# venomouscyanide/S3GRL

Hardware: AMD Instinct MI355X
Metric: link-pair precomputes/sec (higher is better)
Workload: dtype f32; 1 GPU; pubmed_pos_k3; mode=pos, sign_k=3, num_hops=3, num_nodes=19717, features=500, graph=real topology, synthetic features (BASELINE.md §3)

## Files before the change

### s3grl_amd/csrc/s3grl_packed.hip

```cpp
#include <algorithm>
#include <cstdlib>
#include <type_traits>

#include "s3grl_internal.hpp"
#include "s3grl_gather_common.hpp"

namespace s3grl {
namespace {


constexpr int kTile = 512;
constexpr int kWavesPerBlock = 1;

__device__ __forceinline__ int below(uint64_t m) {
  return __builtin_amdgcn_mbcnt_hi((uint32_t)(m >> 32), __builtin_amdgcn_mbcnt_lo((uint32_t)m, 0u));
}

__device__ __forceinline__ float4_t dense_chunk(const float* __restrict__ X, int64_t ld, int F, int64_t row,
                                                int tile, int j) {
  const int col = tile * kTile + j * 4;
  if (col >= F) return (float4_t)(0.f);
  float4_t v = *reinterpret_cast<const float4_t*>(X + row * ld + col);
  if (col + 1 >= F) v.y = 0.f;
  if (col + 2 >= F) v.z = 0.f;
  if (col + 3 >= F) v.w = 0.f;
  return v;
}

__device__ __forceinline__ bool nonzero(float4_t v) {
  return v.x != 0.f || v.y != 0.f || v.z != 0.f || v.w != 0.f;
}

__global__ __launch_bounds__(256) void pk_count_kernel(const float* __restrict__ X, int64_t ld, int F,
                                                       int64_t N, int tiles, int32_t* __restrict__ cnt) {
  const int lane = threadIdx.x & 63;
  const int64_t item = (int64_t)blockIdx.x * 4 + (threadIdx.x >> 6);
  if (item >= N * tiles) return;
  const int tile = (int)(item / N);
  const int64_t row = item - (int64_t)tile * N;
  const uint64_t m0 = __ballot(nonzero(dense_chunk(X, ld, F, row, tile, lane)));
  const uint64_t m1 = __ballot(nonzero(dense_chunk(X, ld, F, row, tile, 64 + lane)));
  if (lane == 0) cnt[item] = __popcll(m0) + __popcll(m1);
}

__global__ __launch_bounds__(256) void pk_fill_kernel(const float* __restrict__ X, int64_t ld, int F,
                                                      int64_t N, int tiles, const int64_t* __restrict__ ptr,
                                                      PackedHdr* __restrict__ hdr,
                                                      float4_t* __restrict__ data) {
  const int lane = threadIdx.x & 63;
  const int64_t item = (int64_t)blockIdx.x * 4 + (threadIdx.x >> 6);
  if (item >= N * tiles) return;
  const int tile = (int)(item / N);
  const int64_t row = item - (int64_t)tile * N;
  const float4_t v0 = dense_chunk(X, ld, F, row, tile, lane);
  const float4_t v1 = dense_chunk(X, ld, F, row, tile, 64 + lane);
  const uint64_t m0 = __ballot(nonzero(v0));
  const uint64_t m1 = __ballot(nonzero(v1));
  const int64_t off = ptr[item] + 1;
  if (item == 0 && lane == 0) data[0] = (float4_t)(0.f);
  if ((m0 >> lane) & 1) data[off + below(m0)] = v0;
  if ((m1 >> lane) & 1) data[off + __popcll(m0) + below(m1)] = v1;
  if (lane == 0) {
    PackedHdr h;
    h.m0 = m0;
    h.m1 = m1;
    h.off = (uint64_t)off;
    h.el = 0;
    hdr[item] = h;
  }
}

typedef unsigned int uint4_t __attribute__((ext_vector_type(4)));
constexpr uint32_t kOobOffset = 0x80000000u;

__device__ __forceinline__ uint32_t select_or_oob(uint64_t mask, uint32_t if_set, uint32_t oob) {
  uint32_t r;
  asm("v_cndmask_b32_e64 %0, %3, %1, %2" : "=v"(r) : "v"(if_set), "s"(mask), "v"(oob));
  return r;
}

template <int K>
__device__ __forceinline__ int el_phase_b_start(const int (&lim)[K], int cnt) {
  constexpr int U = 4;
  int nb = 1;
#pragma unroll
  for (int i = K - 2; i >= 0; --i)
    if (lim[i] == lim[K - 1] && nb == K - 1 - i) nb = K - i;
  if (nb != 1) return cnt;
  const int ngf = cnt / U;
  const int limA = K >= 2 ? lim[K >= 2 ? K - 2 : 0] : 0;
  const int gA = min(ngf, (limA + U - 1) / U);
  return gA < ngf ? gA * U : cnt;
}

typedef unsigned int uint2_t __attribute__((ext_vector_type(2)));

template <int K>
__device__ __forceinline__ void el_phase_b(const Job* __restrict__ jobs, int njobs, const int32_t* __restrict__ c_ids,
                                           const float* __restrict__ c_coef, const float* __restrict__ job_z,
                                           const int32_t* __restrict__ job_lim, const int32_t* __restrict__ job_order,
                                           const PackedHdr* __restrict__ hdr, const ElemEntry* __restrict__ el,
                                           uint32_t el_bytes, int64_t N, const float* __restrict__ X, int64_t ldx,
                                           int F, float* __restrict__ rows_out, float* __restrict__ prows) {
  constexpr int CH = 2;
  constexpr int U = 4;
  constexpr int W = 64;
  const int lane = threadIdx.x & 63;
  const int wid = __builtin_amdgcn_readfirstlane(blockIdx.x * kWavesPerBlock + (threadIdx.x >> 6));
  if (wid >= njobs) return;
  const int jid = __builtin_amdgcn_readfirstlane(job_order[wid]);
  const Job job = jobs[jid];
  if (job.split == 1) return;
  const int cnt = __builtin_amdgcn_readfirstlane(job.support);
  int lim[K];
#pragma unroll
  for (int i = 0; i < K; ++i) lim[i] = __builtin_amdgcn_readfirstlane(job_lim[(int64_t)jid * K + i]);
  const int j0 = el_phase_b_start<K>(lim, cnt);
  if (j0 >= cnt) return;
  float* __restrict__ rows = job.split == 2 ? prows : rows_out;
  const int col0 = blockIdx.y * kTile;
  const int Fp = F + 1;
  const int64_t rstride = (int64_t)(K + 1) * Fp;
  const int nrow = job.node_b >= 0 ? 2 : 1;
  int coff[CH];
  bool cok[CH];
#pragma unroll
  for (int c = 0; c < CH; ++c) {
    coff[c] = col0 + (lane + 64 * c) * 4;
    cok[c] = coff[c] < F;
  }
  float4_t acc[K][2][CH];
#pragma unroll
  for (int i = 0; i < K; ++i)
#pragma unroll
    for (int r = 0; r < 2; ++r)
#pragma unroll
      for (int c = 0; c < CH; ++c) acc[i][r][c] = (float4_t)(0.f);
#pragma unroll
  for (int r = 0; r < 2; ++r) {
    if (r >= nrow) break;
    const float* __restrict__ src = rows + (job.out_row + r) * rstride + (int64_t)K * Fp + 1;
#pragma unroll
    for (int c = 0; c < CH; ++c) {
      if (cok[c]) {
        const int nv = min(4, F - coff[c]);
        if (nv == 4) {
          acc[K - 1][r][c] = *reinterpret_cast<const float4_u*>(src + coff[c]);
        } else {
#pragma unroll
          for (int e = 0; e < 4; ++e)
            if (e < nv) acc[K - 1][r][c][e] = src[coff[c] + e];
        }
      }
    }
  }
  __shared__ __attribute__((aligned(16))) float2 el_lds[2 + kTile];
  float2* const eacc = el_lds + 1;
#pragma unroll
  for (int c = 0; c < CH; ++c)
#pragma unroll
    for (int e = 0; e < 4; ++e) eacc[1 + (lane + 64 * c) * 4 + e] = make_float2(acc[K - 1][0][c][e], acc[K - 1][1][c][e]);
  __syncthreads();

  const uint32_t* __restrict__ uid = reinterpret_cast<const uint32_t*>(c_ids + job.ids_off);
  const float2* __restrict__ cq = reinterpret_cast<const float2*>(c_coef) + job.coef_off + (int64_t)(K - 1) * cnt;
  const PackedHdr* __restrict__ th = hdr + (int64_t)blockIdx.y * N;
  const __amdgpu_buffer_rsrc_t ersrc =
      __builtin_amdgcn_make_buffer_rsrc(const_cast<ElemEntry*>(el), 0, (int)el_bytes, 0x00020000);
  const uint32_t oobv = kOobOffset;
  auto load_e = [&](uint32_t s, uint32_t k, uint32_t n) __attribute__((always_inline)) {
    const uint32_t a = (s + k + (uint32_t)lane) << 3;
    return __builtin_bit_cast(uint2_t, __builtin_amdgcn_raw_buffer_load_b64(
                                           ersrc, (int)(k + (uint32_t)lane < n ? a : oobv), 0, 0));
  };
  auto rmw = [&](uint2_t e, float qx, float qy) __attribute__((always_inline)) {
    float2 a = eacc[e.y];
    const float v = __builtin_bit_cast(float, e.x);
    a.x += qx * v;
    a.y += qy * v;
    eacc[e.y] = a;
  };
  struct EBuf {
    uint2_t e[U];
    uint32_t s[U];
    uint32_t n[U];
  };
  uint32_t idn = j0 + lane < cnt ? uid[j0 + lane] : 0u;
  for (int w0 = j0; w0 < cnt; w0 += W) {
    const int nw = min(W, cnt - w0);
    const bool mine = lane < nw;
    const uint64_t rg = mine ? th[idn].el : 0ull;
    const float2 q = mine ? cq[w0 + lane] : make_float2(0.f, 0.f);
    if (w0 + W + lane < cnt) idn = uid[w0 + W + lane];
    const uint32_t es = (uint32_t)rg, en = (uint32_t)(rg >> 32);
    const int ng = (nw + U - 1) / U;
    auto issue = [&](int g, EBuf& b) __attribute__((always_inline)) {
#pragma unroll
      for (int u = 0; u < U; ++u) {
        const int j = g * U + u;
        const int l = min(j, W - 1);
        b.s[u] = (uint32_t)__builtin_amdgcn_readlane((int)es, l);
        b.n[u] = j < W ? (uint32_t)__builtin_amdgcn_readlane((int)en, l) : 0u;
        b.e[u] = load_e(b.s[u], 0u, b.n[u]);
      }
      __builtin_amdgcn_sched_barrier(0);
    };
    auto rmw_grp = [&](int g, const EBuf& b) __attribute__((always_inline)) {
#pragma unroll
      for (int u = 0; u < U; ++u) {
        const int l = min(g * U + u, W - 1);
        const float qx = __builtin_bit_cast(float, __builtin_amdgcn_readlane(__builtin_bit_cast(int, q.x), l));
        const float qy = __builtin_bit_cast(float, __builtin_amdgcn_readlane(__builtin_bit_cast(int, q.y), l));
        rmw(b.e[u], qx, qy);
        if (__builtin_expect(b.n[u] > 64, 0)) {
#pragma nounroll
          for (uint32_t k = 64; k < b.n[u]; k += 64)
            rmw(load_e(b.s[u], k, b.n[u]), qx, qy);
        }
      }
      __builtin_amdgcn_sched_barrier(0);
    };
    EBuf bA, bB;
    issue(0, bA);
    for (int g = 0; g < ng; g += 2) {
      issue(g + 1, bB);
      rmw_grp(g, bA);
      if (g + 1 < ng) {
        issue(g + 2, bA);
        rmw_grp(g + 1, bB);
      }
    }
  }
  __syncthreads();
#pragma unroll
  for (int c = 0; c < CH; ++c)
#pragma unroll
    for (int e = 0; e < 4; ++e) {
      const float2 a = eacc[1 + (lane + 64 * c) * 4 + e];
      acc[K - 1][0][c][e] = a.x;
      acc[K - 1][1][c][e] = a.y;
    }
  write_pair_rows_part<K, CH, K - 1, K, false, true>(job, jid, acc, coff, cok, job_z, X, ldx, F, rows,
                                                     blockIdx.y == 0);
}

template <int K, int MINNB, int EL>
__global__ __launch_bounds__(kWavesPerBlock * 64) void gather_packed_kernel(
    const Job* __restrict__ jobs, int njobs, const int32_t* __restrict__ c_ids,
    const float* __restrict__ c_coef, const float* __restrict__ job_z,
    const int32_t* __restrict__ job_lim, const int32_t* __restrict__ job_order,
    const PackedHdr* __restrict__ hdr,
    const float4_t* __restrict__ data, uint32_t data_bytes, const ElemEntry* __restrict__ el, uint32_t el_bytes,
    int64_t N, const float* __restrict__ X, int64_t ldx, int F, float* __restrict__ rows_out,
    float* __restrict__ prows) {
  if constexpr (EL == 3) {
    el_phase_b<K>(jobs, njobs, c_ids, c_coef, job_z, job_lim, job_order, hdr, el, el_bytes, N, X, ldx, F, rows_out,
                  prows);
    return;
  }
  constexpr int CH = 2;
  constexpr int U = 4;
  const int lane = threadIdx.x & 63;
  const int wid = __builtin_amdgcn_readfirstlane(blockIdx.x * kWavesPerBlock + (threadIdx.x >> 6));
  if (wid >= njobs) return;
  const int jid = __builtin_amdgcn_readfirstlane(job_order[wid]);
  const int col0 = blockIdx.y * kTile;
  const Job job = jobs[jid];
  if (job.split == 1) return;
  float* __restrict__ rows = job.split == 2 ? prows : rows_out;
  const int cnt = __builtin_amdgcn_readfirstlane(job.support);
  const uint32_t* __restrict__ uid = reinterpret_cast<const uint32_t*>(c_ids + job.ids_off);
  const float2* __restrict__ cf = reinterpret_cast<const float2*>(c_coef) + job.coef_off;
  const PackedHdr* __restrict__ th = hdr + (int64_t)blockIdx.y * N;
  const __amdgpu_buffer_rsrc_t rsrc =
      __builtin_amdgcn_make_buffer_rsrc(const_cast<float4_t*>(data), 0, (int)data_bytes, 0x00020000);
  const uint32_t oobv = kOobOffset;
  int lim[K];
#pragma unroll
  for (int i = 0; i < K; ++i) lim[i] = __builtin_amdgcn_readfirstlane(job_lim[(int64_t)jid * K + i]);

  int coff[CH];
  bool cok[CH];
#pragma unroll
  for (int c = 0; c < CH; ++c) {
    coff[c] = col0 + (lane + 64 * c) * 4;
    cok[c] = coff[c] < F;
  }
  float4_t acc[K][2][CH];
#pragma unroll
  for (int i = 0; i < K; ++i)
#pragma unroll
    for (int r = 0; r < 2; ++r)
#pragma unroll
      for (int c = 0; c < CH; ++c) acc[i][r][c] = (float4_t)(0.f);

  auto hdr_of = [&](uint32_t id) __attribute__((always_inline)) -> PackedHdr {
    static_assert(sizeof(PackedHdr) == 32, "the shift below");
    return *reinterpret_cast<const PackedHdr*>(reinterpret_cast<const char*>(th) + (id << 5));
  };
  auto load_hdrs = [&](int g, PackedHdr(&h)[U]) __attribute__((always_inline)) {
    uint32_t id[U];
#pragma unroll
    for (int u = 0; u < U; ++u) id[u] = uid[g * U + u];
    __builtin_amdgcn_sched_barrier(0);
#pragma unroll
    for (int u = 0; u < U; ++u) h[u] = hdr_of(id[u]);
    __builtin_amdgcn_sched_barrier(0);
  };
  auto load_ids = [&](int g, uint32_t(&id)[U]) __attribute__((always_inline)) {
#pragma unroll
    for (int u = 0; u < U; ++u) id[u] = uid[g * U + u];
    __builtin_amdgcn_sched_barrier(0);
  };
  auto hdrs_from = [&](const uint32_t(&id)[U], PackedHdr(&h)[U]) __attribute__((always_inline)) {
#pragma unroll
    for (int u = 0; u < U; ++u) h[u] = hdr_of(id[u]);
    __builtin_amdgcn_sched_barrier(0);
  };
  auto hdrs_from_late = [&](const uint32_t(&id)[U], PackedHdr(&h)[U]) __attribute__((always_inline)) {
    uint32_t idv[U];
#pragma unroll
    for (int u = 0; u < U; ++u) idv[u] = id[u];
    asm volatile("" : "+s"(idv[0]), "+s"(idv[1]), "+s"(idv[2]), "+s"(idv[3]));
    static_assert(U == 4, "the opaque statement above lists four ids");
#pragma unroll
    for (int u = 0; u < U; ++u) h[u] = hdr_of(idv[u]);
    __builtin_amdgcn_sched_barrier(0);
  };
  auto issue = [&](const PackedHdr(&h)[U], float4_t(&v)[U][CH], bool valid = true) __attribute__((always_inline)) {
#pragma unroll
    for (int u = 0; u < U; ++u) {
      const uint32_t base = valid ? (uint32_t)h[u].off : (kOobOffset >> 4);
      const uint32_t a0 = (base + (uint32_t)below(h[u].m0)) << 4;
      const uint32_t a1 = (base + (uint32_t)__popcll(h[u].m0) + (uint32_t)below(h[u].m1)) << 4;
      v[u][0] = __builtin_bit_cast(float4_t, __builtin_amdgcn_raw_buffer_load_b128(
                                                 rsrc, (int)select_or_oob(h[u].m0, a0, oobv), 0, 0));
      v[u][1] = __builtin_bit_cast(float4_t, __builtin_amdgcn_raw_buffer_load_b128(
                                                 rsrc, (int)select_or_oob(h[u].m1, a1, oobv), 0, 0));
    }
    __builtin_amdgcn_sched_barrier(0);
  };
  auto fma_from = [&](auto first, auto last, int g, const float4_t(&v)[U][CH]) __attribute__((always_inline)) {
    constexpr int I0 = decltype(first)::value, I1 = decltype(last)::value;
#pragma unroll
    for (int i = I0; i < I1; ++i) {
#pragma unroll
      for (int u = 0; u < U; ++u) {
        const float2 q = cf[(int64_t)i * cnt + g * U + u];
#pragma unroll
        for (int c = 0; c < CH; ++c) {
          acc[i][0][c] += q.x * v[u][c];
          acc[i][1][c] += q.y * v[u][c];
        }
      }
    }
  };
  auto tail_rows = [&](auto first, auto last, int j0) __attribute__((always_inline)) {
    constexpr int I0 = decltype(first)::value, I1 = decltype(last)::value;
    for (int j = j0; j < cnt; ++j) {
      const PackedHdr h = hdr_of(uid[j]);
      const uint32_t base = (uint32_t)h.off;
      const uint32_t a0 = (base + (uint32_t)below(h.m0)) << 4;
      const uint32_t a1 = (base + (uint32_t)__popcll(h.m0) + (uint32_t)below(h.m1)) << 4;
      float4_t v[CH];
      v[0] = __builtin_bit_cast(float4_t, __builtin_amdgcn_raw_buffer_load_b128(
                                              rsrc, (int)select_or_oob(h.m0, a0, oobv), 0, 0));
      v[1] = __builtin_bit_cast(float4_t, __builtin_amdgcn_raw_buffer_load_b128(
                                              rsrc, (int)select_or_oob(h.m1, a1, oobv), 0, 0));
#pragma unroll
      for (int i = I0; i < I1; ++i) {
        const float2 q = cf[(int64_t)i * cnt + j];
#pragma unroll
        for (int c = 0; c < CH; ++c) {
          acc[i][0][c] += q.x * v[c];
          acc[i][1][c] += q.y * v[c];
        }
      }
    }
  };

  auto pass2 = [&](auto first, auto last, int g0, int g1) __attribute__((always_inline)) {
    constexpr int I0 = decltype(first)::value;
    constexpr int NO_RAW = decltype(last)::value - I0;
    constexpr int NO = NO_RAW > 0 ? NO_RAW : 1;
    if (NO_RAW <= 0) return;
    if (g1 <= g0) return;
    int g = g0;
    PackedHdr hA[U], hB[U];
    float4_t vA[U][CH], vB[U][CH];
    uint32_t idn[U];
    load_hdrs(g0, hA);
    issue(hA, vA);
    if (g1 - g0 > 1) load_hdrs(g0 + 1, hB);
    if (g1 - g0 > 2) load_ids(g0 + 2, idn);
    float2 qa[NO][U];
    auto load_qa = [&](int gq) {
#pragma unroll
      for (int i = 0; i < NO; ++i)
#pragma unroll
        for (int u = 0; u < U; ++u) qa[i][u] = cf[(int64_t)(I0 + i) * cnt + gq * U + u];
      __builtin_amdgcn_sched_barrier(0);
    };
    auto fma_qa = [&](const float4_t(&v)[U][CH]) {
#pragma unroll
      for (int i = 0; i < NO; ++i)
#pragma unroll
        for (int u = 0; u < U; ++u)
#pragma unroll
          for (int c = 0; c < CH; ++c) {
            acc[I0 + i][0][c] += qa[i][u].x * v[u][c];
            acc[I0 + i][1][c] += qa[i][u].y * v[u][c];
          }
      __builtin_amdgcn_sched_barrier(0);
    };
    auto fma_g = [&](int gq, const float4_t(&v)[U][CH]) {
      fma_from(first, last, gq, v);
      __builtin_amdgcn_sched_barrier(0);
    };
    for (; g + 4 < g1; g += 2) {
      if constexpr (NO <= 3) {
        hdrs_from(idn, hA);
        load_ids(g + 3, idn);
        load_qa(g);
        issue(hB, vB);
        fma_qa(vA);
        hdrs_from(idn, hB);
        load_ids(g + 4, idn);
        load_qa(g + 1);
        issue(hA, vA);
        fma_qa(vB);
      } else {
        issue(hB, vB);
        hdrs_from(idn, hA);
        load_ids(g + 3, idn);
        fma_g(g, vA);
        issue(hA, vA);
        hdrs_from(idn, hB);
        load_ids(g + 4, idn);
        fma_g(g + 1, vB);
      }
    }
    fma_g(g, vA);
    ++g;
    for (; g < g1; ++g) {
      load_hdrs(g, hA);
      issue(hA, vA);
      fma_g(g, vA);
    }
  };

  auto pass3 = [&](int g0, int g1) __attribute__((always_inline)) {
    const int nB = g1 - g0;
    if (nB <= 0) return;
    auto grp = [&](int k) { return g0 + min(k, nB - 1); };
    uint32_t idX[U], idY[U];
    PackedHdr hX[U], hY[U];
    float2 qX[U], qY[U];
    float4_t v0[U][CH], v1[U][CH], v2[U][CH];
    auto load_q = [&](int g, float2(&q)[U]) {
#pragma unroll
      for (int u = 0; u < U; ++u) q[u] = cf[(int64_t)(K - 1) * cnt + g * U + u];
      __builtin_amdgcn_sched_barrier(0);
    };
    auto fma_q = [&](const float2(&q)[U], const float4_t(&v)[U][CH]) {
#pragma unroll
      for (int u = 0; u < U; ++u) {
#pragma unroll
        for (int c = 0; c < CH; ++c) {
          acc[K - 1][0][c] += q[u].x * v[u][c];
          acc[K - 1][1][c] += q[u].y * v[u][c];
        }
      }
      __builtin_amdgcn_sched_barrier(0);
    };
    load_ids(grp(0), idX);
    hdrs_from(idX, hX);
    issue(hX, v0);
    load_ids(grp(1), idX);
    hdrs_from(idX, hY);
    issue(hY, v1, 1 < nB);
    load_ids(grp(2), idX);
    hdrs_from(idX, hX);
    load_ids(grp(3), idX);
    load_q(grp(0), qX);
#define S3GRL_GATHER_STEP(k, IDr, IDl, Hr, Hl, Qr, Ql, Vissue, Vfma) \
  hdrs_from_late(IDr, Hl);                                            \
  load_ids(grp((k) + 4), IDl);                                        \
  load_q(grp((k) + 1), Ql);                                           \
  issue(Hr, Vissue, (k) + 2 < nB);                                    \
  fma_q(Qr, Vfma);
    for (int k = 0; k < nB; k += 6) {
      S3GRL_GATHER_STEP(k, idX, idY, hX, hY, qX, qY, v2, v0)
      S3GRL_GATHER_STEP(k + 1, idY, idX, hY, hX, qY, qX, v0, v1)
      S3GRL_GATHER_STEP(k + 2, idX, idY, hX, hY, qX, qY, v1, v2)
      S3GRL_GATHER_STEP(k + 3, idY, idX, hY, hX, qY, qX, v2, v0)
      S3GRL_GATHER_STEP(k + 4, idX, idY, hX, hY, qX, qY, v0, v1)
      S3GRL_GATHER_STEP(k + 5, idY, idX, hY, hX, qY, qX, v1, v2)
    }
#undef S3GRL_GATHER_STEP
  };

  __shared__ __attribute__((aligned(16))) float2 el_lds[EL == 1 || EL == 2 ? 2 + kTile : 2];
  float2* const eacc = el_lds + 1;
  const __amdgpu_buffer_rsrc_t ersrc =
      __builtin_amdgcn_make_buffer_rsrc(const_cast<ElemEntry*>(el), 0, (int)el_bytes, 0x00020000);
  struct EBuf {
    uint2_t e[U];
    uint32_t s[U];
    uint32_t n[U];
  };
  auto issue_e = [&](const PackedHdr(&h)[U], EBuf& b, bool valid) __attribute__((always_inline)) {
#pragma unroll
    for (int u = 0; u < U; ++u) {
      b.s[u] = (uint32_t)h[u].el;
      b.n[u] = valid ? (uint32_t)(h[u].el >> 32) : 0u;
      const uint32_t a = (b.s[u] + (uint32_t)lane) << 3;
      b.e[u] = __builtin_bit_cast(uint2_t, __builtin_amdgcn_raw_buffer_load_b64(
                                               ersrc, (int)((uint32_t)lane < b.n[u] ? a : oobv), 0, 0));
    }
    __builtin_amdgcn_sched_barrier(0);
  };
  auto rmw = [&](uint2_t e, float2 q) __attribute__((always_inline)) {
    float2 a = eacc[e.y];
    const float v = __builtin_bit_cast(float, e.x);
    a.x += q.x * v;
    a.y += q.y * v;
    eacc[e.y] = a;
  };
  auto rmw_row = [&](uint2_t e, uint32_t s, uint32_t n, float2 q) __attribute__((always_inline)) {
    rmw(e, q);
    if (__builtin_expect(n <= 64, 1)) return;
#pragma nounroll
    for (uint32_t k = 64; k < n; k += 64) {
      const uint32_t a = (s + k + (uint32_t)lane) << 3;
      const uint2_t t = __builtin_bit_cast(uint2_t, __builtin_amdgcn_raw_buffer_load_b64(
                                                        ersrc, (int)(k + (uint32_t)lane < n ? a : oobv), 0, 0));
      rmw(t, q);
    }
  };
  auto pass3e = [&](int g0, int g1) __attribute__((always_inline)) {
    const int nB = g1 - g0;
    if (nB <= 0) return;
    auto grp = [&](int k) { return g0 + min(k, nB - 1); };
    uint32_t idX[U], idY[U];
    PackedHdr hX[U], hY[U];
    float2 qX[U], qY[U];
    EBuf v0, v1, v2;
    auto load_q = [&](int g, float2(&q)[U]) {
#pragma unroll
      for (int u = 0; u < U; ++u) q[u] = cf[(int64_t)(K - 1) * cnt + g * U + u];
      __builtin_amdgcn_sched_barrier(0);
    };
    auto rmw_q = [&](const float2(&q)[U], const EBuf& b) {
#pragma unroll
      for (int u = 0; u < U; ++u) rmw_row(b.e[u], b.s[u], b.n[u], q[u]);
      __builtin_amdgcn_sched_barrier(0);
    };
    load_ids(grp(0), idX);
    hdrs_from(idX, hX);
    issue_e(hX, v0, true);
    load_ids(grp(1), idX);
    hdrs_from(idX, hY);
    issue_e(hY, v1, 1 < nB);
    load_ids(grp(2), idX);
    hdrs_from(idX, hX);
    load_ids(grp(3), idX);
    load_q(grp(0), qX);
#define S3GRL_GATHER_STEP(k, IDr, IDl, Hr, Hl, Qr, Ql, Vissue, Vrmw) \
  hdrs_from_late(IDr, Hl);                                            \
  load_ids(grp((k) + 4), IDl);                                        \
  load_q(grp((k) + 1), Ql);                                           \
  issue_e(Hr, Vissue, (k) + 2 < nB);                                  \
  if ((k) < nB) rmw_q(Qr, Vrmw);
    for (int k = 0; k < nB; k += 6) {
      S3GRL_GATHER_STEP(k, idX, idY, hX, hY, qX, qY, v2, v0)
      S3GRL_GATHER_STEP(k + 1, idY, idX, hY, hX, qY, qX, v0, v1)
      S3GRL_GATHER_STEP(k + 2, idX, idY, hX, hY, qX, qY, v1, v2)
      S3GRL_GATHER_STEP(k + 3, idY, idX, hY, hX, qY, qX, v2, v0)
      S3GRL_GATHER_STEP(k + 4, idX, idY, hX, hY, qX, qY, v0, v1)
      S3GRL_GATHER_STEP(k + 5, idY, idX, hY, hX, qY, qX, v1, v2)
    }
#undef S3GRL_GATHER_STEP
  };
  auto tail_rows_e = [&](int j0) __attribute__((always_inline)) {
    for (int j = j0; j < cnt; ++j) {
      const PackedHdr h = hdr_of(uid[j]);
      const uint32_t es = (uint32_t)h.el, en = (uint32_t)(h.el >> 32);
      const uint2_t e = __builtin_bit_cast(uint2_t, __builtin_amdgcn_raw_buffer_load_b64(
                                                        ersrc, (int)((uint32_t)lane < en ? (es + (uint32_t)lane) << 3 : oobv), 0, 0));
      rmw_row(e, es, en, cf[(int64_t)(K - 1) * cnt + j]);
    }
  };
  auto acc_to_lds = [&]() __attribute__((always_inline)) {
#pragma unroll
    for (int c = 0; c < CH; ++c)
#pragma unroll
      for (int e = 0; e < 4; ++e) eacc[1 + (lane + 64 * c) * 4 + e] = make_float2(acc[K - 1][0][c][e], acc[K - 1][1][c][e]);
    __syncthreads();
  };
  auto lds_to_acc = [&]() __attribute__((always_inline)) {
    __syncthreads();
#pragma unroll
    for (int c = 0; c < CH; ++c)
#pragma unroll
      for (int e = 0; e < 4; ++e) {
        const float2 a = eacc[1 + (lane + 64 * c) * 4 + e];
        acc[K - 1][0][c][e] = a.x;
        acc[K - 1][1][c][e] = a.y;
      }
  };

  const int ngf = cnt / U;
  auto run = [&](auto nb_c) __attribute__((always_inline)) {
    constexpr int NB = decltype(nb_c)::value;
    using IC0 = std::integral_constant<int, 0>;
    using ICS = std::integral_constant<int, K - NB>;
    using ICK = std::integral_constant<int, K>;
    const int limA = NB < K ? lim[NB < K ? K - NB - 1 : 0] : 0;
    const int gA = min(ngf, (limA + U - 1) / U);
    const bool tail_in_A = limA > ngf * U;
    if constexpr (NB == 1) {
      pass2(IC0{}, ICK{}, 0, gA);
      if (tail_in_A) tail_rows(IC0{}, ICK{}, ngf * U);
      write_pair_rows_part<K, CH, 0, K - NB, true, false>(job, jid, acc, coff, cok, job_z, X, ldx, F, rows,
                                                          blockIdx.y == 0);
      __builtin_amdgcn_sched_barrier(0);
      if constexpr (EL == 2) {
        if (gA < ngf) {
          Job jp = job;
          jp.mirror_row = -1;
          write_pair_rows_part<K, CH, K - 1, K, false, false>(jp, jid, acc, coff, cok, job_z, X, ldx, F, rows,
                                                              false);
          return;
        }
        acc_to_lds();
        if (!tail_in_A) tail_rows_e(ngf * U);
        lds_to_acc();
      } else if constexpr (EL == 1) {
        acc_to_lds();
        pass3e(gA, ngf);
        if (!tail_in_A) tail_rows_e(ngf * U);
        lds_to_acc();
      } else {
        pass3(gA, ngf);
        if (!tail_in_A) tail_rows(ICS{}, ICK{}, ngf * U);
      }
    } else {
      pass2(IC0{}, ICS{}, 0, gA);
      if (tail_in_A) tail_rows(IC0{}, ICS{}, ngf * U);
      write_pair_rows_part<K, CH, 0, K - NB, true, false>(job, jid, acc, coff, cok, job_z, X, ldx, F, rows,
                                                          blockIdx.y == 0);
      __builtin_amdgcn_sched_barrier(0);
      pass2(ICS{}, ICK{}, 0, ngf);
      tail_rows(ICS{}, ICK{}, ngf * U);
    }
    write_pair_rows_part<K, CH, K - NB, K, false, true>(job, jid, acc, coff, cok, job_z, X, ldx, F, rows,
                                                        blockIdx.y == 0);
  };
  int nb = 1;
#pragma unroll
  for (int i = K - 2; i >= 0; --i)
    if (lim[i] == lim[K - 1] && nb == K - 1 - i) nb = K - i;
  if constexpr (K >= 3) {
    if (nb >= 3) return run(std::integral_constant<int, 3>{});
  }
  if constexpr (K >= 2) {
    if (nb >= 2 || MINNB >= 2) return run(std::integral_constant<int, 2>{});
  }
  if constexpr (MINNB <= 1 || K < 2) run(std::integral_constant<int, 1>{});
}

__global__ __launch_bounds__(256) void gather_traffic_kernel(
    const Job* __restrict__ jobs, int njobs, const int32_t* __restrict__ c_ids,
    const int32_t* __restrict__ job_lim, int K, int packed, int elements, const PackedHdr* __restrict__ hdr,
    int64_t N, int F, int pieces, unsigned long long* __restrict__ out) {
  const int lane = threadIdx.x & 63;
  const int jid = blockIdx.x * 4 + (threadIdx.x >> 6);
  if (jid >= njobs) return;
  const Job job = jobs[jid];
  if (job.split == 1) {
    if (lane == 0) {
      const unsigned long long nr = (job.node_b >= 0 ? 2 : 1) * (job.mirror_row >= 0 ? 2 : 1);
      atomicAdd(&out[4], 4ull * nr * (K + 1) * (unsigned long long)(F + 1));
      atomicAdd(&out[5], 16ull * ((F + 3) / 4) * (job.node_b >= 0 ? 2 : 1));
    }
    return;
  }
  const int cnt = job.support;
  const int32_t* __restrict__ ids = c_ids + job.ids_off;
  const int tile_cols = packed ? kTile : (F <= 256 ? 256 : 512);
  const int tiles = (F + tile_cols - 1) / tile_cols;
  const unsigned long long chunks_row = (unsigned long long)((F + 3) / 4);
  int nb = 1, nA = 0;
  if (packed) {
    constexpr int U = 4;
    const int ngf = cnt / U;
    for (int i = K - 2; i >= 0; --i)
      if (job_lim[(int64_t)jid * K + i] == job_lim[(int64_t)jid * K + K - 1] && nb == K - 1 - i) nb = K - i;
    nb = min(nb, 3);
    const int limA = nb < K ? job_lim[(int64_t)jid * K + (K - nb - 1)] : 0;
    const int gA = min(ngf, (limA + U - 1) / U);
    const bool tail_in_A = limA > ngf * U;
    nA = tail_in_A ? cnt : gA * U;
  }
  const int twice = (packed && nb >= 2) ? nA : 0;
  const int el_from = (packed && elements && nb == 1) ? nA : cnt;
  const bool split_b = elements == 2 && el_from < cnt / 4 * 4;
  unsigned long long feat = 0;
  if (packed) {
    for (int j = lane; j < cnt; j += 64) {
      const int id = ids[j];
      for (int t = 0; t < tiles; ++t) {
        const PackedHdr h = hdr[(int64_t)t * N + id];
        feat += j >= el_from ? 8ull * (h.el >> 32)
                             : (j < twice ? 32ull : 16ull) * (unsigned long long)(__popcll(h.m0) + __popcll(h.m1));
      }
    }
#pragma unroll
    for (int o = 32; o > 0; o >>= 1) feat += __shfl_xor(feat, o);
  } else {
    feat = 16ull * chunks_row * (unsigned long long)cnt;
  }
  if (lane != 0) return;
  unsigned long long coef_entries = (unsigned long long)K * cnt;
  if (packed)
    coef_entries = nb == 1 ? (unsigned long long)K * nA + (unsigned long long)(cnt - nA)
                           : (unsigned long long)(K - nb) * nA + (unsigned long long)nb * cnt;
  const int nrow = job.node_b >= 0 ? 2 : 1;
  const int ncopy = job.mirror_row >= 0 ? 2 : 1;
  atomicAdd(&out[0], 4ull * (cnt + twice) * tiles);
  atomicAdd(&out[1], packed ? (split_b ? 32ull * el_from + 8ull * (cnt - el_from) : 32ull * (cnt + twice)) * tiles
                            : 0ull);
  atomicAdd(&out[2], feat);
  atomicAdd(&out[3], 8ull * coef_entries * tiles);
  const unsigned long long partial = split_b ? 4ull * nrow * (unsigned long long)F : 0ull;
  atomicAdd(&out[4], 4ull * nrow * ncopy * (K + 1) * (unsigned long long)(F + 1) + partial);
  atomicAdd(&out[5], 16ull * chunks_row * nrow + (pieces ? 4ull * nrow * (K + 1) * (unsigned long long)(F + 1) : 0ull) +
                         partial);
  atomicAdd(&out[6], (unsigned long long)tiles * (sizeof(Job) + 4ull * K + 4ull) * (split_b ? 2ull : 1ull) + 8ull * K);
  atomicAdd(&out[7], (unsigned long long)tiles);
}

constexpr int64_t kSplitMinEntries = 24;
int element_mode(const s3grl_plan* p, const s3grl_features* f) {
  const int depth = p->walk_plan ? 1 : p->cfg.num_hops;
  const int K = p->cfg.sign_k;
  if (!f->packed || !f->elements || (K >= 2 && K - 1 >= depth)) return 0;
  return f->el_nnz >= kSplitMinEntries * f->N * (int64_t)f->tiles ? 2 : 1;
}

template <int K>
s3grl_status launch_packed_k(s3grl_context* ctx, const s3grl_plan* p, const GatherView& v,
                             const s3grl_features* f, float* rows) {
  hipStream_t stream = ctx->stream;
  const unsigned gx = (unsigned)((v.njobs + kWavesPerBlock - 1) / kWavesPerBlock);
  const uint32_t data_bytes = (uint32_t)((f->pk_chunks + 1) * 16);
  const ElemEntry* el = static_cast<const ElemEntry*>(f->el_ent);
  const uint32_t el_bytes = f->elements ? (uint32_t)(f->el_nnz * (int64_t)sizeof(ElemEntry)) : 0u;
  const int depth = p->walk_plan ? 1 : p->cfg.num_hops;
  const int el_mode = element_mode(p, f);
  auto kern = gather_packed_kernel<K, 1, 0>;
  if (K >= 2 && K - 1 >= depth)
    kern = gather_packed_kernel<K, (K >= 2 ? 2 : 1), 0>;
  else if (el_mode == 1)
    kern = gather_packed_kernel<K, 1, 1>;
  else if (el_mode == 2)
    kern = gather_packed_kernel<K, 1, 2>;
  for (int ph = 0; ph < (el_mode == 2 ? 2 : 1); ++ph) {
    const auto kph = ph == 0 ? kern : gather_packed_kernel<K, 1, 3>;
    hipLaunchKernelGGL(kph, dim3(gx, (unsigned)f->tiles),
                       dim3(kWavesPerBlock * 64), 0, stream, v.jobs, (int)v.njobs, p->c_ids, p->c_coef, v.job_z,
                       v.job_lim, v.job_order, static_cast<const PackedHdr*>(f->pk_hdr),
                       static_cast<const float4_t*>(f->pk_data), data_bytes, el, el_bytes, f->N, f->dense, f->ld,
                       (int)f->F, rows, v.prows);
    S3GRL_HIP_TRY(hipGetLastError());
  }
  return S3GRL_OK;
}

}

s3grl_status build_packed_rows(s3grl_context* ctx, s3grl_features* f, double max_density, bool elements) {
  const int64_t N = f->N;
  const int tiles = (int)((f->F + kTile - 1) / kTile);
  const int64_t items = N * tiles;
  Transient tmp{ctx, {}};
  void* q = nullptr;
  S3GRL_TRY(ctx->arena.alloc((size_t)items * 4, &q));
  tmp.ptrs.push_back(q);
  int32_t* cnt = static_cast<int32_t*>(q);
  S3GRL_TRY(ctx->arena.alloc((size_t)(items + 1) * 8, &q));
  tmp.ptrs.push_back(q);
  int64_t* ptr = static_cast<int64_t*>(q);
  S3GRL_TRY(ctx->arena.alloc((size_t)scan_workspace_elems(items) * 8, &q));
  tmp.ptrs.push_back(q);
  int64_t* ws = static_cast<int64_t*>(q);
  const unsigned grid = (unsigned)((items + 3) / 4);
  hipLaunchKernelGGL(pk_count_kernel, dim3(grid), dim3(256), 0, ctx->stream, f->dense, f->ld, (int)f->F, N, tiles, cnt);
  S3GRL_HIP_TRY(hipGetLastError());
  S3GRL_TRY(launch_scan_i32_to_i64(ctx, cnt, items, ptr, ws));
  S3GRL_HIP_TRY(hipMemcpyAsync(ctx->h_scalars, ptr + items, 8, hipMemcpyDeviceToHost, ctx->stream));
  S3GRL_HIP_TRY(hipStreamSynchronize(ctx->stream));
  const int64_t chunks = ctx->h_scalars[0];
  const double slots = (double)N * (double)((f->F + 3) / 4);
  f->pk_chunks = chunks;
  if ((double)chunks > max_density * slots) return S3GRL_OK;
  if ((chunks + 1) * 16 >= ((int64_t)1 << 31)) return S3GRL_OK;
  if (N >= ((int64_t)1 << 27)) return S3GRL_OK;
  void* hdr = nullptr;
  void* data = nullptr;
  S3GRL_TRY(ctx->arena.alloc((size_t)items * sizeof(PackedHdr), &hdr));
  f->owned.push_back(hdr);
  S3GRL_TRY(ctx->arena.alloc((size_t)(chunks + 1) * 16, &data));
  f->owned.push_back(data);
  hipLaunchKernelGGL(pk_fill_kernel, dim3(grid), dim3(256), 0, ctx->stream, f->dense, f->ld, (int)f->F, N, tiles, ptr,
                     static_cast<PackedHdr*>(hdr), static_cast<float4_t*>(data));
  S3GRL_HIP_TRY(hipGetLastError());
  f->pk_hdr = hdr;
  f->pk_data = data;
  f->packed = true;
  if (elements) S3GRL_TRY(build_element_rows(ctx, f));
  return S3GRL_OK;
}

s3grl_status launch_gather_traffic(s3grl_context* ctx, const s3grl_plan* p, const s3grl_features* f,
                                   unsigned long long* d_out) {
  if (p->njobs == 0) return S3GRL_OK;
  if (f->sparse) {
    set_last_error("gather traffic accounting covers the dense and the packed operand");
    return S3GRL_ERR_NOT_IMPLEMENTED;
  }
  const int el = element_mode(p, f);
  hipLaunchKernelGGL(gather_traffic_kernel, dim3((unsigned)((p->njobs + 3) / 4)), dim3(256), 0, ctx->stream,
                     p->jobs, (int)p->njobs, p->c_ids, p->job_lim, p->cfg.sign_k, f->packed ? 1 : 0, el,
                     static_cast<const PackedHdr*>(f->pk_hdr), f->N, (int)f->F, 0, d_out);
  if (p->npieces)
    hipLaunchKernelGGL(gather_traffic_kernel, dim3((unsigned)((p->npieces + 3) / 4)), dim3(256), 0, ctx->stream,
                       p->gjobs + p->njobs, (int)p->npieces, p->c_ids, p->g_lim + p->njobs * p->cfg.sign_k,
                       p->cfg.sign_k, f->packed ? 1 : 0, el, static_cast<const PackedHdr*>(f->pk_hdr), f->N, (int)f->F, 1,
                       d_out);
  S3GRL_HIP_TRY(hipGetLastError());
  return S3GRL_OK;
}

s3grl_status launch_gather_packed(s3grl_context* ctx, const s3grl_plan* p, const GatherView& v,
                                  const s3grl_features* f, float* rows) {
  if (v.njobs == 0) return S3GRL_OK;
  switch (p->cfg.sign_k) {
    case 1: return launch_packed_k<1>(ctx, p, v, f, rows);
    case 2: return launch_packed_k<2>(ctx, p, v, f, rows);
    case 3: return launch_packed_k<3>(ctx, p, v, f, rows);
    case 4: return launch_packed_k<4>(ctx, p, v, f, rows);
    case 5: return launch_packed_k<5>(ctx, p, v, f, rows);
    case 6: return launch_packed_k<6>(ctx, p, v, f, rows);
    case 7: return launch_packed_k<7>(ctx, p, v, f, rows);
    case 8: return launch_packed_k<8>(ctx, p, v, f, rows);
    default:
      set_last_error("sign_k must be in 1..8");
      return S3GRL_ERR_INVALID_ARGUMENT;
  }
}

}

S3GRL_DEFINE_TOUCH(packed)
```

Measured before the change: 15.67 million link pairs/s.

## Stage packed-gather ids and coefficients through LDS records read by readlane

For pass2 with few output hops, the per-group id and coefficient loads are replaced by a cooperative fill that stages a 64-row window of ids and coefficients into LDS records. Each wave then pulls one record dword per lane and extracts scalars with readlane, instead of issuing scattered per-group global loads. The change also adds an amdgpu_waves_per_eu occupancy hint that varies with K, MINNB and EL, and enlarges the shared buffer used for staging. The cost is extra barriers per window refill and more LDS, which may lower occupancy for some variants.

```diff
diff --git a/s3grl_amd/csrc/s3grl_packed.hip b/s3grl_amd/csrc/s3grl_packed.hip
--- a/s3grl_amd/csrc/s3grl_packed.hip
+++ b/s3grl_amd/csrc/s3grl_packed.hip
@@ -11,6 +11,9 @@
 
 constexpr int kTile = 512;
 constexpr int kWavesPerBlock = 1;
+constexpr int kPrefixWindow = 64;
+constexpr int kRecStride = 32;
+constexpr int kStageDwords = kPrefixWindow / 4 * kRecStride + 64;
 
 __device__ __forceinline__ int below(uint64_t m) {
   return __builtin_amdgcn_mbcnt_hi((uint32_t)(m >> 32), __builtin_amdgcn_mbcnt_lo((uint32_t)m, 0u));
@@ -245,7 +248,13 @@
 }
 
 template <int K, int MINNB, int EL>
-__global__ __launch_bounds__(kWavesPerBlock * 64) void gather_packed_kernel(
+constexpr int packed_min_waves() {
+  return EL == 3 ? 8 : (K <= 3 || (MINNB == 2 && K <= 5)) ? 4 : 1;
+}
+
+template <int K, int MINNB, int EL>
+__global__ __launch_bounds__(kWavesPerBlock * 64)
+__attribute__((amdgpu_waves_per_eu(packed_min_waves<K, MINNB, EL>()))) void gather_packed_kernel(
     const Job* __restrict__ jobs, int njobs, const int32_t* __restrict__ c_ids,
     const float* __restrict__ c_coef, const float* __restrict__ job_z,
     const int32_t* __restrict__ job_lim, const int32_t* __restrict__ job_order,
@@ -379,6 +388,9 @@
     }
   };
 
+  __shared__ __attribute__((aligned(16))) float2 el_lds[EL == 1 || EL == 2 ? 2 + kTile : kStageDwords / 2];
+  static_assert(2 * (2 + kTile) >= kStageDwords, "the staging records share the element accumulators' LDS");
+  uint32_t* const stage = reinterpret_cast<uint32_t*>(el_lds);
   auto pass2 = [&](auto first, auto last, int g0, int g1) __attribute__((always_inline)) {
     constexpr int I0 = decltype(first)::value;
     constexpr int NO_RAW = decltype(last)::value - I0;
@@ -386,50 +398,112 @@
     if (NO_RAW <= 0) return;
     if (g1 <= g0) return;
     int g = g0;
-    PackedHdr hA[U], hB[U];
-    float4_t vA[U][CH], vB[U][CH];
-    uint32_t idn[U];
-    load_hdrs(g0, hA);
-    issue(hA, vA);
-    if (g1 - g0 > 1) load_hdrs(g0 + 1, hB);
-    if (g1 - g0 > 2) load_ids(g0 + 2, idn);
-    float2 qa[NO][U];
-    auto load_qa = [&](int gq) {
-#pragma unroll
-      for (int i = 0; i < NO; ++i)
-#pragma unroll
-        for (int u = 0; u < U; ++u) qa[i][u] = cf[(int64_t)(I0 + i) * cnt + gq * U + u];
-      __builtin_amdgcn_sched_barrier(0);
-    };
-    auto fma_qa = [&](const float4_t(&v)[U][CH]) {
-#pragma unroll
-      for (int i = 0; i < NO; ++i)
-#pragma unroll
-        for (int u = 0; u < U; ++u)
-#pragma unroll
-          for (int c = 0; c < CH; ++c) {
-            acc[I0 + i][0][c] += qa[i][u].x * v[u][c];
-            acc[I0 + i][1][c] += qa[i][u].y * v[u][c];
+    if constexpr (NO <= 3) {
+      static_assert(4 + 2 * U * 3 <= kRecStride && kRecStride <= 64, "a record is one dword per lane");
+      constexpr int WG = kPrefixWindow / U;
+      PackedHdr h[U];
+      float4_t vA[U][CH], vB[U][CH];
+      uint32_t rec;
+      const int rlast = g1 * U - 1;
+      auto fill = [&](int gw) __attribute__((always_inline)) {
+        const int r0 = gw * U;
+        const uint32_t oq = (uint32_t)min(lane, rlast - r0);
+        const uint32_t oi = (uint32_t)min(lane + 2 * U, rlast - r0);
+        const uint32_t idv = (uid + r0)[oi];
+        float2 qv[NO];
+#pragma unroll
+        for (int i = 0; i < NO; ++i) qv[i] = (cf + ((int64_t)(I0 + i) * cnt + r0))[oq];
+        __syncthreads();
+        int ll = lane;
+        asm volatile("" : "+v"(ll));
+        uint32_t* const r = stage + (ll >> 2) * kRecStride;
+        r[ll & 3] = idv;
+#pragma unroll
+        for (int i = 0; i < NO; ++i)
+          *reinterpret_cast<uint2_t*>(r + 4 + (i * U + (ll & 3)) * 2) =
+              uint2_t{__builtin_bit_cast(uint32_t, qv[i].x), __builtin_bit_cast(uint32_t, qv[i].y)};
+        __syncthreads();
+        rec = stage[lane];
+        __builtin_amdgcn_sched_barrier(0);
+      };
+      auto ids_at = [&](uint32_t r, int l0, uint32_t(&id)[U]) __attribute__((always_inline)) {
+#pragma unroll
+        for (int u = 0; u < U; ++u) id[u] = (uint32_t)__builtin_amdgcn_readlane((int)r, l0 + u);
+      };
+      auto q_of = [&](float2(&qa)[NO][U]) __attribute__((always_inline)) {
+#pragma unroll
+        for (int i = 0; i < NO; ++i)
+#pragma unroll
+          for (int u = 0; u < U; ++u) {
+            qa[i][u].x = __builtin_bit_cast(float, __builtin_amdgcn_readlane((int)rec, 4 + (i * U + u) * 2));
+            qa[i][u].y = __builtin_bit_cast(float, __builtin_amdgcn_readlane((int)rec, 5 + (i * U + u) * 2));
           }
-      __builtin_amdgcn_sched_barrier(0);
-    };
-    auto fma_g = [&](int gq, const float4_t(&v)[U][CH]) {
-      fma_from(first, last, gq, v);
-      __builtin_amdgcn_sched_barrier(0);
-    };
-    for (; g + 4 < g1; g += 2) {
-      if constexpr (NO <= 3) {
-        hdrs_from(idn, hA);
-        load_ids(g + 3, idn);
-        load_qa(g);
-        issue(hB, vB);
-        fma_qa(vA);
-        hdrs_from(idn, hB);
-        load_ids(g + 4, idn);
-        load_qa(g + 1);
-        issue(hA, vA);
-        fma_qa(vB);
-      } else {
+      };
+      auto fma_rec = [&](const float2(&qa)[NO][U], const float4_t(&v)[U][CH]) __attribute__((always_inline)) {
+#pragma unroll
+        for (int u = 0; u < U; ++u) {
+#pragma unroll
+          for (int i = 0; i < NO; ++i)
+#pragma unroll
+            for (int c = 0; c < CH; ++c) {
+              acc[I0 + i][0][c] += qa[i][u].x * v[u][c];
+              acc[I0 + i][1][c] += qa[i][u].y * v[u][c];
+            }
+          __builtin_amdgcn_sched_barrier(0);
+        }
+      };
+      auto half = [&](int snext, float4_t(&vi)[U][CH], bool valid, const float4_t(&vf)[U][CH]) __attribute__((always_inline)) {
+        issue(h, vi, valid);
+        uint32_t id[U];
+        float2 qa[NO][U];
+        ids_at(rec, 0, id);
+        q_of(qa);
+        __builtin_amdgcn_sched_barrier(0);
+        hdrs_from(id, h);
+        rec = stage[snext * kRecStride + lane];
+        __builtin_amdgcn_sched_barrier(0);
+        fma_rec(qa, vf);
+      };
+      {
+        const uint32_t id0v = (uid + g0 * U)[(uint32_t)min(lane, min(2 * U - 1, rlast - g0 * U))];
+        fill(g0);
+        uint32_t id[U];
+        ids_at(id0v, 0, id);
+        hdrs_from(id, h);
+        issue(h, vA);
+        ids_at(id0v, U, id);
+        hdrs_from(id, h);
+      }
+      int s = 0;
+      for (; g + 1 < g1; g += 2) {
+        if (s == WG) {
+          fill(g);
+          s = 0;
+        }
+        half(s + 1, vB, true, vA);
+        half(s + 2, vA, g + 2 < g1, vB);
+        s += 2;
+      }
+      if (g < g1) {
+        if (s == WG) fill(g);
+        float2 qa[NO][U];
+        q_of(qa);
+        __builtin_amdgcn_sched_barrier(0);
+        fma_rec(qa, vA);
+      }
+    } else {
+      PackedHdr hA[U], hB[U];
+      float4_t vA[U][CH], vB[U][CH];
+      uint32_t idn[U];
+      load_hdrs(g0, hA);
+      issue(hA, vA);
+      if (g1 - g0 > 1) load_hdrs(g0 + 1, hB);
+      if (g1 - g0 > 2) load_ids(g0 + 2, idn);
+      auto fma_g = [&](int gq, const float4_t(&v)[U][CH]) {
+        fma_from(first, last, gq, v);
+        __builtin_amdgcn_sched_barrier(0);
+      };
+      for (; g + 4 < g1; g += 2) {
         issue(hB, vB);
         hdrs_from(idn, hA);
         load_ids(g + 3, idn);
@@ -439,13 +513,13 @@
         load_ids(g + 4, idn);
         fma_g(g + 1, vB);
       }
-    }
-    fma_g(g, vA);
-    ++g;
-    for (; g < g1; ++g) {
-      load_hdrs(g, hA);
-      issue(hA, vA);
       fma_g(g, vA);
+      ++g;
+      for (; g < g1; ++g) {
+        load_hdrs(g, hA);
+        issue(hA, vA);
+        fma_g(g, vA);
+      }
     }
   };
 
@@ -500,7 +574,6 @@
 #undef S3GRL_GATHER_STEP
   };
 
-  __shared__ __attribute__((aligned(16))) float2 el_lds[EL == 1 || EL == 2 ? 2 + kTile : 2];
   float2* const eacc = el_lds + 1;
   const __amdgpu_buffer_rsrc_t ersrc =
       __builtin_amdgcn_make_buffer_rsrc(const_cast<ElemEntry*>(el), 0, (int)el_bytes, 0x00020000);
```

Measured after the change: 16.05 million link pairs/s (median of 6 runs). +2.4%, better.
